# richardshuai/ExPecto

Measured on AMD Instinct MI355X. Metric: variants/sec (200 windows × 2002 feats) at 1/2/4/8 MI355X; HBM GB/s vs peak, higher is better.
Workload: dtype fp32 in/out (f16x3: power-of-2-scaled 2-way fp16 split = 22-bit operands, 3 MFMA products, fp32 accumulate; bf16x6 recompute on fp16 overflow)

## Files before the change

### expecto_amd/csrc/beluga.hip

```cpp
#include <hip/hip_runtime.h>

#include <algorithm>
#include <array>
#include <cstdint>
#include <cstdlib>
#include <cstring>
#include <map>
#include <memory>
#include <mutex>
#include <tuple>
#include <string>
#include <vector>

#include "beluga_knobs.h"
#include "common.h"
#include "event_pairs.h"
#include "gemm_kernel.h"
#include "seg_plan.h"

namespace expecto {

static_assert(kStrandFwd == EXPECTO_STRAND_FWD && kStrandRc == EXPECTO_STRAND_RC && kStrandBoth == EXPECTO_STRAND_BOTH &&
              EXPECTO_EINVAL == -1, "seg_plan.h restates the strand modes and the refusal code");
constexpr int kNFeat = 2002;
// ... 155 lines not shown
#pragma unroll
        for (int j = 0; j < 4; ++j) {
          const float v = fmaxf(fmaf(acc[rb][cb][j], sc[cb], bb[cb]), 0.f);
          vmax = fmaxf(vmax, v);
          _Float16 h, l;
          split_h2p(v, h, l);
          char* d = sw + (16 * rb + 4 * fq + j) * C1H_WROW + (cb >> 1) * 128 + ((cb & 1) * 16 + fr) * 2;
          *reinterpret_cast<_Float16*>(d) = h;
          *reinterpret_cast<_Float16*>(d + 64) = l;
        }
    asm volatile("s_waitcnt lgkmcnt(0)" ::: "memory");
#pragma unroll
    for (int i = 0; i < (C1H_STEP * 16) / 64; ++i) {
      const int k = i * 64 + lane, row = k >> 4, ch = k & 15;
      if (s + row < tend) {
        char* g = reinterpret_cast<char*>(out) + ((win * out_rows + t0 + s + row) * 10 + 2 * wave) * 128 + ch * 16;
        *reinterpret_cast<floatx4*>(g) = *reinterpret_cast<const floatx4*>(sw + row * C1H_WROW + ch * 16);
      }
    }
    asm volatile("s_waitcnt lgkmcnt(0)" ::: "memory");
  }
  if ((bad || !(vmax < 65504.f)) && ovf) *ovf = 1;
}

__global__ void fc1_reduce(const float* __restrict__ part, int splits, long long split_stride, long long count,
                           const float* __restrict__ bias, float* __restrict__ h1, int fmt,
                           const float* __restrict__ col_scale, float osc, int* __restrict__ ovf) {
  const long long i = (long long)blockIdx.x * blockDim.x + threadIdx.x;
  if (i >= count) return;
  const long long row = i / kHidLd;
  const int n = (int)(i - row * kHidLd);
  float s = 0.f;
  for (int k = 0; k < splits; ++k) s += part[k * split_stride + i];
  if (col_scale) s *= col_scale[n];
  const float v = n < kFc1Out ? fmaxf(s + bias[n], 0.f) : 0.f;
  store_act_rt(fmt, h1, row, kHidLd, n, v, osc, ovf);
}

typedef _Float16 halfx4 __attribute__((ext_vector_type(4)));
__global__ void fc1_reduce_h2(const float* __restrict__ part, int splits, long long split_stride, long long count4,
                              const float* __restrict__ bias, float* __restrict__ h1,
                              const float* __restrict__ col_scale, float osc, int* __restrict__ ovf) {
  const long long i4 = (long long)blockIdx.x * blockDim.x + threadIdx.x;
  if (i4 >= count4) return;
  const long long i = i4 * 4;
  const long long row = i / kHidLd;
  const int n = (int)(i - row * kHidLd);
  floatx4 s = {0.f, 0.f, 0.f, 0.f};
  for (int k = 0; k < splits; ++k) {
    const floatx4 v = *reinterpret_cast<const floatx4*>(part + k * split_stride + i);
#pragma unroll
    for (int e = 0; e < 4; ++e) s[e] += v[e];
  }
  halfx4 hv, lv;
  bool bad = false;
#pragma unroll
  for (int e = 0; e < 4; ++e) {
    float t = s[e];
    if (col_scale) t *= col_scale[n + e];
    const float v = n + e < kFc1Out ? fmaxf(t + bias[min(n + e, kFc1Out - 1)], 0.f) : 0.f;
    const float x = v * osc;
    bad |= !(fabsf(x) < 65504.f);
    _Float16 hh, ll;
    split_h2p(x, hh, ll);
    hv[e] = hh;
    lv[e] = ll;
  }
  if (bad && ovf) *ovf = 1;
  _Float16* d = reinterpret_cast<_Float16*>(h1) + act_index<2>(row, kHidLd, n);
  *reinterpret_cast<halfx4*>(d) = hv;
  *reinterpret_cast<halfx4*>(d + 32) = lv;
}

constexpr int kFc2Chunk = 8;
__device__ __forceinline__ float fc2_value(float s, const float* __restrict__ col_scale, const float* __restrict__ bias,
                                           int n) {
  if (col_scale) s *= col_scale[n];
  const float v = s + bias[n];
  return 1.0f / (1.0f + expf(-v));
}
__global__ __launch_bounds__(256) void fc2_reduce(const float* __restrict__ part, int splits, long long split_stride,
                                                  int M, const float* __restrict__ bias,
                                                  const float* __restrict__ col_scale,
                                                  const long long* __restrict__ c_rows, float* __restrict__ y) {
  static_assert(kNFeat % 2 == 0 && kHidLd % 2 == 0, "2 features per thread");
  const int n = 2 * (blockIdx.x * blockDim.x + threadIdx.x);
  if (n >= kNFeat) return;
  for (long long m = blockIdx.y; m < M; m += gridDim.y) {
    const float* src = part + m * kHidLd + n;
    float s0 = 0.f, s1 = 0.f;
    for (int k0 = 0; k0 < splits; k0 += kFc2Chunk) {
      float2 v[kFc2Chunk];
#pragma unroll
      for (int u = 0; u < kFc2Chunk; ++u)
        v[u] = *reinterpret_cast<const float2*>(src + (long long)min(k0 + u, splits - 1) * split_stride);
#pragma unroll
      for (int u = 0; u < kFc2Chunk; ++u)
        if (k0 + u < splits) {
          s0 += v[u].x;
          s1 += v[u].y;
        }
    }
    float2 o;
    o.x = fc2_value(s0, col_scale, bias, n);
    o.y = fc2_value(s1, col_scale, bias, n + 1);
    *reinterpret_cast<float2*>(y + (c_rows ? c_rows[m] : m) * kNFeat + n) = o;
  }
}
__global__ void fc2_reduce1(const float* __restrict__ part, int splits, long long split_stride, int M,
                            const float* __restrict__ bias, const float* __restrict__ col_scale,
                            const long long* __restrict__ c_rows, float* __restrict__ y) {
  const long long i = (long long)blockIdx.x * blockDim.x + threadIdx.x;
  if (i >= (long long)M * kNFeat) return;
  const int m = (int)(i / kNFeat), n = (int)(i - (long long)m * kNFeat);
  const long long src = (long long)m * kHidLd + n;
  float s = 0.f;
  for (int k = 0; k < splits; ++k) s += part[k * split_stride + src];
  y[(c_rows ? c_rows[m] : m) * kNFeat + n] = fc2_value(s, col_scale, bias, n);
}

__global__ void pool4_phases(const float* __restrict__ in, int n_seg, int s_in, int t_in, int C,
                             int n_ph, int4 ph, int s_out, float* __restrict__ out, int fmt) {
  const int c = threadIdx.x;
  const int g = blockIdx.x;
  const int i = blockIdx.y % n_ph;
  const long long seg = blockIdx.y / n_ph;
  const int p = i == 0 ? ph.x : i == 1 ? ph.y : i == 2 ? ph.z : ph.w;
  if (c >= C || g >= (t_in - p) / 4) return;
  const long long r0 = seg * s_in + p + 4LL * g, orow = (seg * n_ph + i) * s_out + g;
  float m = load_act_rt(fmt, in, r0, C, c);
#pragma unroll
  for (int j = 1; j < 4; ++j) m = fmaxf(m, load_act_rt(fmt, in, r0 + j, C, c));
  store_act_rt(fmt, out, orow, C, c, m);
}

typedef _Float16 halfx8 __attribute__((ext_vector_type(8)));
__global__ __launch_bounds__(256) void pool4_phases_h2(const float* __restrict__ in, int s_in, int t_in, int C,
                                                        int n_ph, int4 ph, int s_out, float* __restrict__ out) {
  const int c8 = threadIdx.x & 63;
  const int g = blockIdx.x * 4 + (threadIdx.x >> 6);
  const int i = blockIdx.y % n_ph;
  const long long seg = blockIdx.y / n_ph;
  const int p = i == 0 ? ph.x : i == 1 ? ph.y : i == 2 ? ph.z : ph.w;
  if (c8 >= C / 8 || g >= (t_in - p) / 4) return;
  const long long rb = (long long)C * 4;
  const int cofs = (c8 >> 2) * 128 + (c8 & 3) * 16;
  const char* src = reinterpret_cast<const char*>(in) + (seg * s_in + p + 4LL * g) * rb + cofs;
  halfx8 hi[4], lo[4];
#pragma unroll
  for (int j = 0; j < 4; ++j) {
    hi[j] = *reinterpret_cast<const halfx8*>(src + j * rb);
    lo[j] = *reinterpret_cast<const halfx8*>(src + j * rb + 64);
  }
  halfx8 oh, ol;
#pragma unroll
  for (int e = 0; e < 8; ++e) {
    float m = (float)hi[0][e] + (float)lo[0][e];
#pragma unroll
    for (int j = 1; j < 4; ++j) m = fmaxf(m, (float)hi[j][e] + (float)lo[j][e]);
    _Float16 h, l;
    split_h2(m, h, l);
    oh[e] = h;
    ol[e] = l;
  }
  char* dst = reinterpret_cast<char*>(out) + ((seg * n_ph + i) * s_out + g) * rb + cofs;
  *reinterpret_cast<halfx8*>(dst) = oh;
  *reinterpret_cast<halfx8*>(dst + 64) = ol;
}

__global__ __launch_bounds__(256) void pool4_phases_h2m(const float* __restrict__ in, int s_in, int t_in, int C,
                                                         int n_ph, int4 ph, int s_out, float* __restrict__ out) {
  const int c8 = threadIdx.x & 63;
  const int g = blockIdx.x * 4 + (threadIdx.x >> 6);
  const long long seg = blockIdx.y;
  const int pmin = ph.x;
  const int pmax = n_ph == 1 ? ph.x : n_ph == 2 ? ph.y : n_ph == 3 ? ph.z : ph.w;
  if (c8 >= C / 8 || g >= (t_in - pmin) / 4) return;
  const long long rb = (long long)C * 4;
  const int cofs = (c8 >> 2) * 128 + (c8 & 3) * 16;
  const char* src = reinterpret_cast<const char*>(in) + (seg * s_in + pmin + 4LL * g) * rb + cofs;
  const int nr = min(pmax - pmin + 4, t_in - pmin - 4 * g);
  halfx8 hi[7], lo[7];
#pragma unroll
  for (int j = 0; j < 7; ++j) {
    if (j < nr) {
      hi[j] = *reinterpret_cast<const halfx8*>(src + j * rb);
      lo[j] = *reinterpret_cast<const halfx8*>(src + j * rb + 64);
    }
  }
  float fv[7][8];
#pragma unroll
  for (int j = 0; j < 7; ++j)
#pragma unroll
    for (int e = 0; e < 8; ++e) fv[j][e] = j < nr ? (float)hi[j][e] + (float)lo[j][e] : 0.f;
#pragma unroll
  for (int i = 0; i < 4; ++i) {
    if (i >= n_ph) break;
    const int p = i == 0 ? ph.x : i == 1 ? ph.y : i == 2 ? ph.z : ph.w;
    if (g >= (t_in - p) / 4) continue;
    const int o = p - pmin;
    halfx8 oh, ol;
// ... 1557 lines not shown
      beluga_conv_h3p<4, EPI_POOL_PH02, 256, 4><<<dim3((unsigned)nblk), dim3(512), 0, st>>>(a);
    if ((rc = check_launch("beluga_conv_h3p pool2"))) return rc;
  }
  Timer lt(h, 3, st);
  if (a.m_tiles > 1)
    pool2_tile_seams<<<dim3((unsigned)(a.m_tiles - 1)), dim3(64), 0, st>>>(h->seam, a.M, s_in, t4, s5, dst);
  return check_launch("pool2_tile_seams");
}

float* h1_rows(expecto_beluga* h, long long rows) { return h->h1 + rows * kHidLd * act_bytes() / 4; }

bool fc_wide_tiles(const expecto_beluga* h) { return h->fc_wide && g_precision == EXPECTO_PRECISION_F16X3; }

bool fc1_narrow(const expecto_beluga* h, long long mtt);
bool fc_skinny(const expecto_beluga* h, long long rows);

int run_fc1(expecto_beluga* h, const float* act, const long long* a_rows, int nb, float* h1, hipStream_t st,
            const unsigned* ks_mask = nullptr, double slab_frac = 1.0, long long part_rows = 0) {
  if (part_rows <= 0) part_rows = nb;
  int rc;
  const long long m_tiles = (nb + gemm_bm() - 1) / gemm_bm();
  const bool wide = fc_wide_tiles(h);
  const int n_tiles1 = wide ? (kHidLd + FCW_BN - 1) / FCW_BN : npad_of(kFc1Out) / GBN;
  const int splits = h->fc_splits;
  {
    GemmArgs a{};
    a.A = act;
    a.a_rows = a_rows;
    a.lda = (long long)kFc1In;
    a.M = nb;
    a.B = h->fc1w;
    a.Bp = g_precision == EXPECTO_PRECISION_F16X3 ? h->wh[5] : h->fc1p;
    a.ldb = kFc1In;
    a.kper = kFc1In / splits;
    a.taps = 1;
    a.n_tiles = n_tiles1;
    a.m_tiles = m_tiles;
    a.m_fastest = (double)m_tiles * gemm_bm() * (kFc1In / splits) * 4.0 <= h->fc1_m_order_mb * (1 << 20) ? 1 : 0;
    a.linear_order = a.m_fastest;
    if (h->fc1_order == 2 && !a.m_fastest && m_tiles % 8 == 0 && planes_gemm() && g_precision == EXPECTO_PRECISION_F16X3)
      a.m_fastest = 2;
    if (h->fc1_order == 3 && g_precision == EXPECTO_PRECISION_F16X3) {
      a.m_fastest = 3;
      a.m_group = h->fc1_m_group;
      a.linear_order = 0;
    }
    if (wide) {
      a.m_fastest = 0;
      a.linear_order = 0;
      a.n_tile_cols = FCW_BN;
      if (!ks_mask && fc_skinny(h, nb)) {
        a.n_tile_cols = 16 * FCS_NB;
        a.n_tiles = kHidLd / a.n_tile_cols;
      } else if (!ks_mask && fc1_narrow(h, m_tiles * splits)) {
        a.n_tile_cols = 112;
        a.n_tiles = kHidLd / 112;
      }
    }
    a.C = h->part;
    a.ldc = kHidLd;
    a.n_store = kHidLd;
    a.split_stride = part_rows * kHidLd;
    a.ks_mask = ks_mask;
    EXPECTO_REQUIRE(!ks_mask || planes_gemm(), "slab mask needs the planes GEMM");
    Timer lt(h, 6, st);
    if (h->profiling) h->macs[h->timer_base + 6] += (double)nb * kFc1Out * kFc1In * slab_frac;
    if ((rc = launch_gemm<7, EPI_PARTIAL>(a, splits, st))) return rc;
  }
  {
    Timer lt(h, 7, st);
    const long long count = (long long)nb * kHidLd;
    const bool f16 = g_precision == EXPECTO_PRECISION_F16X3;
    if (act_fmt() == 2)
      fc1_reduce_h2<<<dim3((unsigned)((count / 4 + 255) / 256)), dim3(256), 0, st>>>(
          h->part, splits, part_rows * kHidLd, count / 4, h->fc1b, h1, h->cs[5], exp2i(h->sx[6]), h->ovf);
    else
      fc1_reduce<<<dim3((unsigned)((count + 255) / 256)), dim3(256), 0, st>>>(
          h->part, splits, part_rows * kHidLd, count, h->fc1b, h1, act_fmt(), f16 ? h->cs[5] : nullptr, exp2i(h->sx[6]), h->ovf);
    if ((rc = check_launch("fc1_reduce"))) return rc;
  }
  return EXPECTO_OK;
}

int run_fc2(expecto_beluga* h, const float* h1, int nb, float* y, hipStream_t st, const long long* c_rows) {
  int rc;
  const long long m_tiles = (nb + gemm_bm() - 1) / gemm_bm();
  {
    GemmArgs a{};
    a.A = h1;
    a.lda = kHidLd;
    a.M = nb;
    a.B = h->fc2w;
    a.Bp = g_precision == EXPECTO_PRECISION_F16X3 ? h->wh[6] : h->fc2p;
    a.col_scale = g_precision == EXPECTO_PRECISION_F16X3 ? h->cs[6] : nullptr;
    a.ldb = kHidLd;
    a.kper = kHidLd / h->fc2_splits;
    a.taps = 1;
    const bool wide = fc_wide_tiles(h) && h->fc2_splits > 1;
    a.n_tiles = wide ? (kNFeat + FCW_BN - 1) / FCW_BN : npad_of(kNFeat) / GBN;
    a.m_tiles = m_tiles;
    a.m_fastest = (double)m_tiles * gemm_bm() * (kHidLd / h->fc2_splits) * 4.0 <= h->fc1_m_order_mb * (1 << 20) ? 1 : 0;
    if (wide) {
      a.m_fastest = 0;
      a.n_tile_cols = FCW_BN;
      if (fc_skinny(h, nb)) {
        a.n_tile_cols = 16 * FCS_NB;
        a.n_tiles = (kNFeat + a.n_tile_cols - 1) / a.n_tile_cols;
      } else if (fc1_narrow(h, m_tiles * h->fc2_splits)) {
        a.n_tile_cols = 112;
        a.n_tiles = (kNFeat + 111) / 112;
      }
    }
    a.C = h->part2;
    a.ldc = kHidLd;
    a.n_store = kNFeat;
    a.split_stride = (long long)nb * kHidLd;
    Timer lt(h, 8, st);
    if (h->profiling) h->macs[h->timer_base + 8] += (double)nb * kNFeat * kFc1Out;
    if (h->fc2_splits == 1) {
      a.C = y;
      a.ldc = kNFeat;
      a.c_rows = c_rows;
      a.bias = h->fc2b;
      a.s_in = a.t_valid = a.s_out = 1;
      return launch_gemm<8, EPI_SIGMOID>(a, 1, st);
    }
    if ((rc = launch_gemm<8, EPI_PARTIAL>(a, h->fc2_splits, st))) return rc;
    if ((reinterpret_cast<uintptr_t>(y) & 7) == 0)
      fc2_reduce<<<dim3((unsigned)((kNFeat / 2 + 255) / 256), (unsigned)std::max<long long>(1, std::min<long long>(nb, 65535))), dim3(256), 0,
                   st>>>(h->part2, h->fc2_splits, (long long)nb * kHidLd, nb, h->fc2b, a.col_scale, c_rows, y);
    else
      fc2_reduce1<<<dim3((unsigned)(((long long)nb * kNFeat + 255) / 256)), dim3(256), 0, st>>>(
          h->part2, h->fc2_splits, (long long)nb * kHidLd, nb, h->fc2b, a.col_scale, c_rows, y);
    if ((rc = check_launch("fc2_reduce"))) return rc;
  }
  return EXPECTO_OK;
}

int run_fc(expecto_beluga* h, const float* act, const long long* a_rows, int nb, float* y, hipStream_t st,
           const long long* c_rows = nullptr, const unsigned* ks_mask = nullptr, double slab_frac = 1.0,
           long long part_rows = 0) {
  int rc;
  if ((rc = run_fc1(h, act, a_rows, nb, h->h1, st, ks_mask, slab_frac, part_rows))) return rc;
  return run_fc2(h, h->h1, nb, y, st, c_rows);
}

int count_desc_macs(expecto_beluga* h, const unsigned* mask, int tiles, double per_tile, hipStream_t st);

bool fk_use(const expecto_beluga* h) {
  return h->fk_on && h->fkw && g_precision == EXPECTO_PRECISION_F16X3 && h->fk_role < 4;
}
bool fk_use_seg(const expecto_beluga* h) { return h->fk_on && h->fkw && g_precision == EXPECTO_PRECISION_F16X3; }

int fk_cap(const expecto_beluga* h) {
  const long long dflt = std::min<long long>((long long)kFkSlicePerBatch * h->max_batch, 1LL << 30);
  return std::max(h->max_batch, h->fk_slice ? h->fk_slice : (int)dflt);
}
constexpr int kGresPerBatch = 3;

int fk_tables(expecto_beluga* h) {
  if (h->fk_grows) return EXPECTO_OK;
  const size_t mb = h->max_batch, tiles = (mb + 255) / 256, cap = fk_cap(h);
  float *a = nullptr, *b = nullptr, *c = nullptr, *d = nullptr;
  int rc;
  if ((rc = dalloc(h, &a, 2 * 9 * cap)) || (rc = dalloc(h, &b, 2 * mb)) || (rc = dalloc(h, &c, kFkParts * cap)) ||
      (rc = dalloc(h, &d, kFkParts * tiles)))
    return rc;
  h->fk_grows = reinterpret_cast<long long*>(a);
  h->fk_wrows = reinterpret_cast<long long*>(b);
  h->fk_prow = reinterpret_cast<int*>(c);
  h->fk_mask = reinterpret_cast<unsigned*>(d);
  return EXPECTO_OK;
}

int fk_seg_buffers(expecto_beluga* h) {
  if (h->fk_part) return EXPECTO_OK;
  const size_t cap = fk_cap(h);
  float *a = nullptr, *b = nullptr;
  int rc;
  if ((rc = dalloc(h, &h->fk_part, (size_t)kFkParts * cap * kHidLd)) || (rc = dalloc(h, &h->fk_h1, act_alloc(cap * kHidLd))) ||
      (rc = dalloc(h, &a, 2 * cap)) || (rc = dalloc(h, &b, 2 * cap)))
    return rc;
  h->fk_arows = reinterpret_cast<long long*>(a);
  h->fk_crows = reinterpret_cast<long long*>(b);
  float *c = nullptr, *d = nullptr, *e = nullptr, *f = nullptr, *q = nullptr, *m = nullptr;
  if ((rc = dalloc(h, &c, 9 * cap)) || (rc = dalloc(h, &d, 2 * cap)) || (rc = dalloc(h, &e, 2 * cap)) ||
      (rc = dalloc(h, &f, kFkParts * cap)) || (rc = dalloc(h, &q, cap)) || (rc = dalloc(h, &m, 19 * (cap / 256 + 1))))
    return rc;
  h->fk_rgrp = reinterpret_cast<int*>(c);
  h->fk_ginfo = reinterpret_cast<int*>(d);
  h->fk_winfo = reinterpret_cast<int*>(e);
  h->fk_aprow = reinterpret_cast<int*>(f);
  h->fk_aperm = reinterpret_cast<int*>(q);
  h->fk_smask = reinterpret_cast<unsigned*>(m);
  return EXPECTO_OK;
}

int fk_seq_alloc(expecto_beluga* h, long long rows, int set = 0) {
  int rc = EXPECTO_OK;
  for (DevBuf<float>& b : set ? h->fk_aseq : h->fk_seq)
    if ((rc = b.reserve(((size_t)rows + 16) * 640, h->bytes))) break;
  return rc;
}

int fk_sequences(expecto_beluga* h, const float* x, long long blocks, int T, int s, const int* tab, int n_ph,
                 hipStream_t st, const int* gres = nullptr, int set = 0) {
  int rc;
  if ((rc = fk_seq_alloc(h, blocks * s, set))) return rc;
  const DevBuf<float>* out = set ? h->fk_aseq : h->fk_seq;
  Timer lt(h, 7, st);
  const long long nblk = blocks * 7;
  EXPECTO_REQUIRE(nblk > 0 && nblk < (1LL << 31), "FC1 sequence grid");
  fk_seq_h2<<<dim3((unsigned)nblk), dim3(320), 0, st>>>(x, T, s, tab, n_ph, gres, out[0], out[1], out[2], h->ovf);
  return check_launch("fk_seq_h2");
}

// ... 266 lines not shown
  if ((rc = dalloc(h, &h->DA, act_alloc(da))) || (rc = dalloc(h, &h->D0, act_alloc(dd))) ||
      (rc = dalloc(h, &h->D1, act_alloc(dd))) || (rc = dalloc(h, &pc, (size_t)h->max_batch * kC1PatStride / 4)) ||
      (rc = dalloc(h, &tb, (size_t)h->max_batch * kSegTab)) ||
      (rc = dalloc(h, &h->slab_mask, (size_t)h->max_batch / 64 + 64)))
    return rc;
  h->delta_codes = reinterpret_cast<uint8_t*>(pc);
  h->seg_tab = reinterpret_cast<int*>(tb);
  if (h->overlap) {
    EXPECTO_HIP_CHECK(hipStreamCreateWithFlags(&h->st2, hipStreamNonBlocking));
    for (hipEvent_t& e : h->pev) EXPECTO_HIP_CHECK(hipEventCreateWithFlags(&e, hipEventDisableTiming));
  }
  return EXPECTO_OK;
}

struct SegPairs {
  const int* var_pos;
  const uint8_t* alt_code;
  float* y_alt;
  long long strand_stride;
};

struct SegCall {
  expecto_beluga* h;
  const SegPlan& pl;
  hipStream_t st, sa;
  const SegPairs* pr;
  SegDims gd;
  int4 ph4, phi;
  int eb;
  const uint8_t* codes;
  long long code_stride;
  int mode;
  float* y;
  const int* win_row_d;
};
struct SegChunk {
  size_t ci;
  int s0, ns, w0, nw;
  long long nb;
};
struct PQSwap {
  expecto_beluga* h;
  bool on;
  ~PQSwap() {
    if (on) std::swap(h->P, h->Q);
  }
};

int stream_order(hipStream_t from, hipStream_t to, hipEvent_t e) {
  if (from == to) return EXPECTO_OK;
  EXPECTO_HIP_CHECK(hipEventRecord(e, from));
  EXPECTO_HIP_CHECK(hipStreamWaitEvent(to, e, 0));
  return EXPECTO_OK;
}

int seg_alt_asm(const SegCall& c, const SegChunk& ck, int l, const float* ref, int ref_rows, const float* dprev,
                int wprev, int nbk, int ib, int mult, int irp, int arows, hipEvent_t ready, hipEvent_t done) {
  int rc;
  if ((rc = stream_order(c.st, c.sa, ready))) return rc;
  const int row16 = kConv[l].cin * c.eb / 16;
  seg_delta_assemble<<<dim3(ck.ns * nbk), dim3(256), 0, c.sa>>>(ref, ref_rows, dprev, wprev, c.h->seg_tab, nbk, ib,
                                                                 mult, irp, arows, row16, c.h->DA);
  rc = check_launch("seg_delta_assemble");
  if (!rc && c.sa != c.st) EXPECTO_HIP_CHECK(hipEventRecord(done, c.sa));
  return rc;
}
int seg_alt_gemm(const SegCall& c, const SegChunk& ck, int l, int nbk, int arows, int w, bool pool, float* dnext) {
  DeltaScope ds(c.h);
  return run_conv(c.h, l, c.h->DA, dnext, (long long)ck.ns * nbk, arows, w, w, pool, c.sa);
}
int seg_st_wait(const SegCall& c, hipEvent_t e) {
  if (c.sa != c.st) EXPECTO_HIP_CHECK(hipStreamWaitEvent(c.st, e, 0));
  return EXPECTO_OK;
}

int seg_rows(const SegCall& c, const SegChunk& ck, const int* widx, int w0, int n, long long* a_rows,
             long long* c_rows) {
  seg_a_rows<<<dim3((n + 255) / 256), dim3(256), 0, c.st>>>(c.h->win_seg_d, c.h->win_off_d, c.win_row_d, widx, w0, n,
                                                             ck.s0, c.pl.ss, c.pl.g.L, c.pl.n_ph, c.phi, c.pl.g.T6,
                                                             a_rows, c_rows);
  return check_launch("seg_a_rows");
}

int seg_fc2(const SegCall& c, const float* h1, int n, float* y, const long long* c_rows) {
  int rc;
  for (int r0 = 0; r0 < n; r0 += c.h->max_batch)
    if ((rc = run_fc2(c.h, h1 + (long long)r0 * kHidLd, std::min(c.h->max_batch, n - r0), y, c.st, c_rows + r0)))
      return rc;
  return EXPECTO_OK;
}

int seg_alt_conv6(const SegCall& c, const SegChunk& ck, bool on_sa = false) {
  int rc;
  const hipStream_t s = on_sa ? c.sa : c.st;
  if ((rc = s == c.st ? seg_st_wait(c, c.h->pev[13]) : stream_order(c.st, s, c.h->pev[14]))) return rc;
  seg_alt_blocks<<<dim3(kAltRows6, (unsigned)ck.nb), dim3(64), 0, s>>>(c.h->P, c.h->D0, c.pl.n_ph, c.pl.g.T6,
                                                                        c.h->seg_tab, 640 * c.eb / 16, c.h->Q);
  return check_launch("seg_alt_blocks");
}

int seg_copy_tail(const SegCall& c, const SegChunk& ck) {
  if (!c.pr) return EXPECTO_OK;
  const std::vector<int>& cw = c.pl.copy_w;
  const int ic0 = (int)(std::lower_bound(cw.begin(), cw.end(), ck.w0) - cw.begin());
  const int ic1 = (int)(std::lower_bound(cw.begin(), cw.end(), ck.w0 + ck.nw) - cw.begin());
  if (ic1 <= ic0) return EXPECTO_OK;
  copy_rows<<<dim3(ic1 - ic0), dim3(256), 0, c.st>>>(c.y, c.pr->y_alt, c.h->copy_w_d + ic0, c.win_row_d, c.pl.ss.n_win,
                                                      c.pl.ss.rc_rows);
  return check_launch("copy_rows");
}

int seg_trunk(const SegCall& c, const SegChunk& ck, PQSwap& pq) {
  expecto_beluga* h = c.h;
  const SegPairs* pr = c.pr;
  const SegGeo& g = c.pl.g;
  const hipStream_t st = c.st, sa = c.sa;
  const int s0 = ck.s0, ns = ck.ns, n_ph = c.pl.n_ph;
  const long long nb = ck.nb;
  int rc;
  if (pr && (rc = stream_order(st, sa, h->pev[0]))) return rc;
  const bool kmer = use_kmer(h, nullptr);
  const bool fuse = !kmer && fuse_conv1(h, nullptr);
  const C1Src f1{c.codes, c.code_stride, c.pl.ss.n_seg, c.mode, s0, g.L};
  if (!kmer && !fuse &&
      (rc = run_conv1(h, nullptr, c.codes, c.code_stride, c.pl.ss.n_seg, c.mode, s0, ns, g.L, g.S1, st)))
    return rc;
  if (pr) {
    seg_delta_table<<<dim3((ns + 255) / 256), dim3(256), 0, sa>>>(h->seg_var_d, s0, ns, c.pl.ss, c.gd, n_ph, c.ph4,
                                                                 h->seg_tab);
    if ((rc = check_launch("seg_delta_table"))) return rc;
    if (kmer || fuse) {
      seg_delta_codes2<<<dim3((ns + 4) / 5), dim3(5 * kC1PatStride), 0, sa>>>(
          c.codes, c.code_stride, pr->alt_code, s0, ns, c.pl.ss, g.L, h->seg_tab, h->delta_codes);
      if ((rc = check_launch("seg_delta_codes2"))) return rc;
      DeltaScope ds(h);
      if (fuse && (rc = run_conv1(h, nullptr, h->delta_codes, kC1PatStride, ns, EXPECTO_STRAND_FWD, 0, ns, kC1Pat,
                                  kDA[2], sa, h->DA)))
        return rc;
    } else {
      seg_delta_codes<<<dim3((ns + 15) / 16), dim3(256), 0, sa>>>(c.codes, c.code_stride, pr->alt_code, s0, ns,
                                                                 c.pl.ss, g.L, h->seg_tab, h->delta_codes);
      if ((rc = check_launch("seg_delta_codes"))) return rc;
      DeltaScope ds(h);
      if ((rc = run_conv1(h, nullptr, h->delta_codes, 16, ns, EXPECTO_STRAND_FWD, 0, ns, kDA[1], kDW[1], sa, h->D0)))
        return rc;
    }
  }
  if (pr && !kmer && !fuse &&
      (rc = seg_alt_asm(c, ck, 0, h->P, g.S1, h->D0, kDW[1], 1, 2, 4, 1, kDA[2], h->pev[1], h->pev[2])))
    return rc;
  if (kmer)
    rc = run_conv2_kmer(h, f1, ns, g.P1, g.P1, h->Q, st);
  else
    rc = run_conv(h, 0, h->P, h->Q, ns, g.S1, g.P1, g.P1, true, st, fuse ? &f1 : nullptr);
  if (rc) return rc;
  if (pr && kmer) {
    DeltaScope ds(h);
    const C1Src fa{h->delta_codes, kC1PatStride, ns, EXPECTO_STRAND_FWD, 0, kC1Pat};
    if ((rc = run_conv2_kmer(h, fa, ns, kDW[2], kDW[2], h->D1, sa))) return rc;
  } else if (pr && ((!fuse && (rc = seg_st_wait(c, h->pev[2]))) ||
                    (rc = seg_alt_gemm(c, ck, 0, 1, kDA[2], kDW[2], true, h->D1)))) {
    return rc;
  }
  if (pr && (rc = seg_alt_asm(c, ck, 1, h->Q, g.P1, h->D1, kDW[2], 1, 3, 1, 2, kDA[3], h->pev[3], h->pev[4])))
    return rc;
  const int T3p = (g.T3 + 3) & ~3;
  if ((rc = run_conv(h, 1, h->Q, h->P, ns, g.P1, g.T3, T3p, false, st))) return rc;
  if (pr && ((rc = seg_st_wait(c, h->pev[4])) || (rc = seg_alt_gemm(c, ck, 1, 1, kDA[3], kDW[3], false, h->D0))))
    return rc;
  if (pr && (rc = seg_alt_asm(c, ck, 2, h->P, T3p, h->D0, kDW[3], 1, 4, 1, 3, kA4u, h->pev[5], h->pev[6])))
    return rc;
// ... 123 lines not shown
  t.rows = row + (long long)ap.tail.size() - row0;
  const int fn = (int)(sl.i1 - sl.i0);
  for (int i = 0; i < fn; ++i) t.perm.push_back(ws[sl.i0 + i].w);
  auto pos_in = [](const std::vector<int>& l, int v) {
    const auto it = std::lower_bound(l.begin(), l.end(), v);
    return it != l.end() && *it == v ? (int)(it - l.begin()) : -1;
  };
  int k = -1;
  size_t next = 0;
  for (size_t i = 0; i < sl.nw_pre && next < ap.win.size(); ++i) {
    if (i == 0 || !fk_same_group(ws[sl.i0 + i], ws[sl.i0 + i - 1])) ++k;
    if ((int)i != ap.win[next]) continue;
    ++next;
    const FkWin& w = ws[sl.i0 + i];
    t.perm.push_back(w.w);
    const size_t p0 = prow.size();
    prow.resize(p0 + kFkParts);
    for (int j = 0; j < kFkParts; ++j) prow[p0 + j] = prow[i * kFkParts + j];
    for (int j = 0; j < 4; ++j) {
      const int g = kFkRole[fk_role_of(w.off6)][j];
      for (int sb = 0; sb < kFkSlabs; ++sb) {
        const int at = pos_in(ap.grp[g][sb], k);
        if (at >= 0) prow[p0 + kFkSlabs * j + sb] = (int)(base[g][sb] + at);
      }
    }
    const int at = pos_in(ap.tail, (int)i);
    if (at >= 0) prow[p0 + kFkParts - 1] = (int)(tail_base + at);
  }
  return t;
}

int seg_fc_karatsuba(const SegCall& c, const SegChunk& ck) {
  expecto_beluga* h = c.h;
  const SegPlan& pl = c.pl;
  const hipStream_t st = c.st;
  const int T6 = pl.g.T6, n_ph = pl.n_ph;
  const long long nb = ck.nb, cap = pl.fk_cap;
  const std::vector<FkWin>& ws = pl.fk_ref[ck.ci];
  const int* perm = h->fc_perm_d + ck.w0;
  int rc;
  const std::vector<int> gres = pl.fk_gres(ck.ci);
  EXPECTO_REQUIRE(nb <= kGresPerBatch * (long long)h->max_batch, "conv6 blocks of a chunk exceed fk_gres");
  if ((rc = stage_copies(h, {{h->fk_gres, gres.data(), gres.size() * sizeof(int)}}, st)) || (rc = fk_tables(h)) ||
      (rc = fk_seg_buffers(h)))
    return rc;
  bool alt_ready = false;
  const bool alt_early = c.pr && !h->fk_alt_inplace && !pl.fk_alt[ck.ci].empty();
  if (alt_early) {
    if ((rc = seg_alt_sequences(c, ck, true))) return rc;
    alt_ready = true;
  }
  if ((rc = fk_sequences(h, h->P, nb, T6, T6, nullptr, n_ph, st, h->fk_gres))) return rc;
  if (alt_early && (rc = seg_st_wait(c, h->pev[15]))) return rc;
  FkSlice sl{};
  for (size_t i0 = 0; i0 < ws.size(); i0 = sl.i1) {
    const char* refusal = pl.fk_slice(ck.ci, i0, sl);
    EXPECTO_REQUIRE(!refusal, refusal);
    const int fn = (int)(sl.i1 - i0);
    std::vector<long long> grows;
    std::vector<int> prow, rgrp, ginfo;
    FkProducts prd{h->fk_grows, {}, {}, {}};
    fk_slice_tables(ws, (int)i0, (int)sl.i1, T6, grows, prd, prow, &rgrp, &ginfo);
    if (sl.n_ag > 0 && !h->fk_alt_inplace) {
      const FkAltPlan ap = pl.fk_alt_plan(ck.ci, sl);
      const int na = (int)ap.win.size();
      long long ref_rows = fn, alt_lists = (long long)ap.tail.size();
      for (int g = 0; g < 9; ++g) {
        ref_rows += (long long)kFkSlabs * prd.cnt[g];
        for (int sb = 0; sb < kFkSlabs; ++sb) alt_lists += (long long)ap.grp[g][sb].size();
      }
      if (fn + na <= cap && ref_rows + alt_lists <= kFkParts * cap && (long long)grows.size() + alt_lists <= 9 * cap) {
        FkAltRowTables t = fk_alt_row_tables(ws, sl, ap, T6, ref_rows, grows, prow);
        t.ar.x = h->Q;
        t.ar.seq = h->fk_aseq;
        t.ar.g_rows = h->fk_grows;
        t.ar.w_rows = h->fk_grows + t.w_off;
        if ((rc = stage_copies(h, {{h->fk_grows, grows.data(), grows.size() * sizeof(long long)},
                                   {h->fk_prow, prow.data(), prow.size() * sizeof(int)},
                                   {h->fk_aperm, t.perm.data(), t.perm.size() * sizeof(int)}}, st)) ||
            (rc = seg_rows(c, ck, h->fk_aperm, 0, fn + na, h->fk_arows, h->fk_crows)) ||
            (rc = fk_fc1(h, h->P, h->fk_seq, prd, h->fk_arows, fn, nullptr, h->fk_h1, st, nullptr, 0, h->fk_part,
                         kFkParts * cap, &t.ar)) ||
            (rc = fk_reduce(h, h->fk_part, h->fk_prow, fn + na, h->fk_h1, st)) ||
            (rc = seg_fc2(c, h->fk_h1, fn, c.y, h->fk_crows)) ||
            (na > 0 && (rc = seg_fc2(c, h->fk_h1 + (long long)fn * kHidLd, na, c.pr->y_alt, h->fk_crows + fn))))
          return rc;
        continue;
      }
    }
    if ((rc = stage_copies(h, {{h->fk_grows, grows.data(), grows.size() * sizeof(long long)},
                               {h->fk_prow, prow.data(), prow.size() * sizeof(int)}}, st)) ||
        (rc = seg_rows(c, ck, perm + i0, 0, fn, h->fk_arows, h->fk_crows)) ||
        (rc = fk_fc1(h, h->P, h->fk_seq, prd, h->fk_arows, fn, h->fk_prow, h->fk_h1, st, nullptr, 0, h->fk_part,
                     kFkParts * cap)) ||
        (rc = seg_fc2(c, h->fk_h1, fn, c.y, h->fk_crows)))
      return rc;
    if (sl.n_ag == 0) continue;
    const FkAltTables t = fk_alt_tables(pl, ws, sl, prd, rgrp, prow);
    const int na = (int)t.aperm.size();
    const int tiles = (int)(cap / 256 + 1);
    if ((rc = stage_copies(h, {{h->fk_rgrp, rgrp.data(), rgrp.size() * sizeof(int)},
                               {h->fk_ginfo, ginfo.data(), ginfo.size() * sizeof(int)},
                               {h->fk_winfo, t.winfo.data(), t.winfo.size() * sizeof(int)},
                               {h->fk_aperm, t.aperm.data(), t.aperm.size() * sizeof(int)},
                               {h->fk_aprow, t.aprow.data(), t.aprow.size() * sizeof(int)}}, st)))
      return rc;
    if (!alt_ready) {
      if ((rc = seg_alt_sequences(c, ck, false))) return rc;
      alt_ready = true;
    }
    EXPECTO_HIP_CHECK(hipMemsetAsync(h->fk_smask, 0, (size_t)(t.md.n + 1) * tiles * sizeof(unsigned), st));
    int rows_max = t.md.nw;
    for (int i = 0; i < t.md.n; ++i) rows_max = std::max(rows_max, t.md.cnt[i]);
    if (rows_max > 0) {
      fk_seg_mask<<<dim3((rows_max + 255) / 256, t.md.n + 1), dim3(256), 0, st>>>(
          t.md, h->fk_rgrp, h->fk_ginfo, h->fk_winfo, h->seg_tab, n_ph, make_int4(0, 0, 0, 0), tiles, h->fk_smask);
      if ((rc = check_launch("fk_seg_mask"))) return rc;
    }
    DeltaScope ds(h);
    if ((rc = fk_fc1(h, h->Q, h->fk_aseq, t.pa, h->fk_arows, (int)sl.nw_pre, nullptr, h->fk_h1, st, h->fk_smask, tiles,
                     h->fk_part, kFkParts * cap)) ||
        (na > 0 && ((rc = fk_reduce(h, h->fk_part, h->fk_aprow, na, h->fk_h1, st)) ||
                    (rc = seg_rows(c, ck, h->fk_aperm, 0, na, h->fk_arows, h->fk_crows)) ||
                    (rc = seg_fc2(c, h->fk_h1, na, c.pr->y_alt, h->fk_crows)))))
      return rc;
  }
  return seg_copy_tail(c, ck);
}

int seg_fc_direct(const SegCall& c, const SegChunk& ck) {
  expecto_beluga* h = c.h;
  const SegPairs* pr = c.pr;
  const SegPlan& pl = c.pl;
  const hipStream_t st = c.st;
  const int w0 = ck.w0, nw = ck.nw;
  int rc;
  const int* widx = pr ? h->fc_perm_d + w0 : nullptr;
  const int n_alt = !pr ? 0 : (int)(std::lower_bound(pl.alt_w.begin(), pl.alt_w.end(), w0 + nw) -
                                    std::lower_bound(pl.alt_w.begin(), pl.alt_w.end(), w0));
  const bool gather2 = h->fc2_splits == 1;
  int pend = 0;
  auto flush2 = [&]() -> int {
    const int n2 = pend;
    pend = 0;
    return n2 ? run_fc2(h, h->h1, n2, c.y, st, h->c_rows) : EXPECTO_OK;
  };
  for (int f0 = 0; f0 < nw; f0 += h->max_batch) {
    const int fn = std::min(h->max_batch, nw - f0);
    if (gather2 && pend + fn > h->fc2_rows && (rc = flush2())) return rc;
    long long* crow = h->c_rows + (gather2 ? pend : 0);
    if ((rc = seg_rows(c, ck, widx ? widx + f0 : nullptr, w0 + f0, fn, h->a_rows, crow))) return rc;
    if (gather2) {
      if ((rc = run_fc1(h, h->P, h->a_rows, fn, h1_rows(h, pend), st))) return rc;
      pend += fn;
    } else if ((rc = run_fc(h, h->P, h->a_rows, fn, c.y, st, h->c_rows))) {
      return rc;
    }
    const int na = std::min(n_alt - f0, fn);
    if (na <= 0) continue;
    if (f0 == 0 && (rc = seg_alt_conv6(c, ck))) return rc;
    long long* acrow = gather2 ? h->c_rows + h->fc2_rows : h->c_rows;
    if ((rc = seg_rows(c, ck, widx + f0, 0, na, h->a_rows, acrow))) return rc;
    const unsigned* mask = nullptr;
    double frac = 1.0;
    if (planes_gemm()) {
      const int tiles = (int)((na + gemm_bm() - 1) / gemm_bm());
      unsigned* md = reinterpret_cast<unsigned*>(h->slab_mask);
      EXPECTO_HIP_CHECK(hipMemsetAsync(md, 0, tiles * sizeof(unsigned), st));
      fc1_slab_mask_seg<<<dim3((na + 255) / 256), dim3(256), 0, st>>>(
          widx + f0, na, h->win_seg_d, h->win_off_d, ck.s0, pl.ss, pl.g.L, c.phi, h->seg_tab, (int)gemm_bm(),
          kFc1In / h->fc_splits, md);
      if ((rc = check_launch("fc1_slab_mask_seg"))) return rc;
      mask = md;
      if (h->profiling) {
        if ((rc = count_slab_macs(h, md, tiles, na, st))) return rc;
        frac = 0.0;
      }
    }
    DeltaScope ds(h);
    if (gather2) {
      float* h1a = h1_rows(h, h->fc2_rows);
      if ((rc = run_fc1(h, h->Q, h->a_rows, na, h1a, st, mask, frac, fn)) ||
          (rc = run_fc2(h, h1a, na, pr->y_alt, st, acrow)))
        return rc;
    } else if ((rc = run_fc(h, h->Q, h->a_rows, na, pr->y_alt, st, h->c_rows, mask, frac, fn))) {
      return rc;
    }
  }
  if ((rc = flush2())) return rc;
  return seg_copy_tail(c, ck);
}

int forward_segments(expecto_beluga* h, const uint8_t* codes, int n_seg, int L, long long code_stride, int mode,
                     const int* win_seg, const int* win_off, const int* win_row, int n_win, float* y,
                     hipStream_t st, const SegPairs* pr = nullptr) {
  g_precision = h->precision;
  g_conv_ea = h->conv_ea;
  SegPlan pl;
  const char* refusal = nullptr;
  if (seg_plan({n_seg, L, mode, win_seg, win_off, win_row, n_win, pr ? pr->var_pos : nullptr,
                pr ? pr->strand_stride : n_win, h->max_batch, p_floats(h->max_batch) - 16 * 640,
                q_floats(h->max_batch) - 16 * 640, h->seg_merge_strands, h->seg_chunk_windows, fk_use_seg(h), fk_cap(h),
                h->fk_alt_inplace},
               pl, &refusal)) {
    set_error(refusal);
    return EXPECTO_EINVAL;
  }
// ... 702 lines not shown
```

### expecto_amd/csrc/beluga_knobs.h

```cpp
#pragma once

#include <algorithm>
#include <cstdlib>
#include <limits>

namespace expecto {

constexpr int kFc1KBlocks = 2120;
constexpr int kFc2KBlocks = 63;
constexpr int kFc2SplitsDefault = 7;
constexpr int kFcSplitsDefault = 8;

constexpr int kFkSlicePerBatch = 5;

struct BelugaKnobs {
  bool overlap = true;
  int fc_splits = kFcSplitsDefault;
  int fc2_splits = kFc2SplitsDefault;
  int fc2_rows_env = 0;
  double fc1_m_order_mb = 80.0;
  int fc1_order = 3;
  int fc1_m_group = 8;
  bool fc_wide = true;
  int conv_tile = 0;
  bool conv_ea = true;
  bool fc_skinny = true;
  int fc1_narrow = -1;
  int conv_narrow = -1;
  int seg_chunk_windows = 0;
  bool seg_merge_strands = true;
  bool pool_one_pass = true;
  bool pool_fused = true;
  bool fuse_conv1 = true;
  bool kmer_on = true;
  bool kmer_quad = true;
  double kmer_max_bytes = std::numeric_limits<double>::infinity();
  bool fk_on = true;
  int fk_role = 4;
  int fk_slice = 0;
  bool fk_alt_inplace = false;
  bool onehot_as_codes = true;
};

struct BelugaKnob {
  const char* name;
  bool BelugaKnobs::*b;
  int BelugaKnobs::*i;
  double BelugaKnobs::*d;
  int floor;
  bool (*ok)(int);
  const char* refusal;
};

namespace knob_detail {
using K = BelugaKnobs;
constexpr int kAny = std::numeric_limits<int>::min();
constexpr BelugaKnob flag(const char* n, bool K::*f) { return {n, f, nullptr, nullptr, kAny, nullptr, nullptr}; }
constexpr BelugaKnob num(const char* n, int K::*f, int floor = kAny, bool (*ok)(int) = nullptr, const char* why = nullptr) {
  return {n, nullptr, f, nullptr, floor, ok, why};
}
constexpr BelugaKnob real(const char* n, double K::*f) { return {n, nullptr, nullptr, f, kAny, nullptr, nullptr}; }
inline bool fc1_splits_ok(int v) { return v >= 1 && v <= 32 && kFc1KBlocks % v == 0; }
inline bool fc2_splits_ok(int v) { return v >= 1 && kFc2KBlocks % v == 0; }
inline bool role_ok(int v) { return v >= 0 && v <= 4; }
inline bool tri_ok(int v) { return v >= -1 && v <= 1; }
inline bool conv_tile_ok(int v) { return v == 0 || v == 256 || v == 384; }
}

inline constexpr BelugaKnob kBelugaKnobs[] = {
    knob_detail::num("EXPECTO_FC1_SPLITS", &BelugaKnobs::fc_splits, knob_detail::kAny, knob_detail::fc1_splits_ok,
                     "EXPECTO_FC1_SPLITS must divide 2120 and be <= 32"),
    knob_detail::num("EXPECTO_FC2_SPLITS", &BelugaKnobs::fc2_splits, knob_detail::kAny, knob_detail::fc2_splits_ok,
                     "EXPECTO_FC2_SPLITS must divide 63"),
    knob_detail::num("EXPECTO_FC2_ROWS", &BelugaKnobs::fc2_rows_env, 1),
    knob_detail::real("EXPECTO_FC1_M_ORDER_MB", &BelugaKnobs::fc1_m_order_mb),
    knob_detail::num("EXPECTO_FC1_ORDER", &BelugaKnobs::fc1_order),
    knob_detail::num("EXPECTO_FC1_M_GROUP", &BelugaKnobs::fc1_m_group, 1),
    knob_detail::flag("EXPECTO_FC_WIDE", &BelugaKnobs::fc_wide),
    knob_detail::flag("EXPECTO_OVERLAP", &BelugaKnobs::overlap),
    knob_detail::flag("EXPECTO_POOL_ONE_PASS", &BelugaKnobs::pool_one_pass),
    knob_detail::flag("EXPECTO_POOL_FUSED", &BelugaKnobs::pool_fused),
    knob_detail::flag("EXPECTO_FUSE_CONV1", &BelugaKnobs::fuse_conv1),
    knob_detail::flag("EXPECTO_CONV2_TABLE", &BelugaKnobs::kmer_on),
    knob_detail::flag("EXPECTO_KMER_QUAD", &BelugaKnobs::kmer_quad),
    knob_detail::real("EXPECTO_KMER_MAX_BYTES", &BelugaKnobs::kmer_max_bytes),
    knob_detail::flag("EXPECTO_ONEHOT_CODES", &BelugaKnobs::onehot_as_codes),
    knob_detail::flag("EXPECTO_FC1_KARATSUBA", &BelugaKnobs::fk_on),
    knob_detail::num("EXPECTO_FC1K_SLICE", &BelugaKnobs::fk_slice, 1),
    knob_detail::num("EXPECTO_FC1_ROLE", &BelugaKnobs::fk_role, knob_detail::kAny, knob_detail::role_ok,
                     "EXPECTO_FC1_ROLE must be 0..4"),
    knob_detail::num("EXPECTO_SEG_CHUNK_WINDOWS", &BelugaKnobs::seg_chunk_windows),
    knob_detail::flag("EXPECTO_SEG_MERGE_STRANDS", &BelugaKnobs::seg_merge_strands),
    knob_detail::num("EXPECTO_CONV_NARROW", &BelugaKnobs::conv_narrow, knob_detail::kAny, knob_detail::tri_ok,
                     "EXPECTO_CONV_NARROW must be -1 (auto), 0 or 1"),
    knob_detail::num("EXPECTO_FC1_NARROW", &BelugaKnobs::fc1_narrow, knob_detail::kAny, knob_detail::tri_ok,
                     "EXPECTO_FC1_NARROW must be -1 (auto), 0 or 1"),
    knob_detail::flag("EXPECTO_CONV_EA", &BelugaKnobs::conv_ea),
    knob_detail::flag("EXPECTO_FC_SKINNY", &BelugaKnobs::fc_skinny),
    knob_detail::num("EXPECTO_CONV_TILE", &BelugaKnobs::conv_tile, knob_detail::kAny, knob_detail::conv_tile_ok,
                     "EXPECTO_CONV_TILE must be 0 (auto), 256 or 384"),
};

inline constexpr BelugaKnob kBelugaSwitches[] = {
    knob_detail::flag("EXPECTO_FC1K_ALT_INPLACE", &BelugaKnobs::fk_alt_inplace),
};

template <class Getenv>
const char* beluga_knobs_parse(BelugaKnobs& k, Getenv&& get) {
  for (const BelugaKnob& s : kBelugaKnobs) {
    const char* e = get(s.name);
    if (!e) continue;
    if (s.b) {
      k.*s.b = atoi(e) != 0;
    } else if (s.d) {
      k.*s.d = atof(e);
    } else {
      const int v = std::max(s.floor, atoi(e));
      if (s.ok && !s.ok(v)) return s.refusal;
      k.*s.i = v;
    }
  }
  for (const BelugaKnob& s : kBelugaSwitches)
    if (const char* e = get(s.name)) k.*s.b = atoi(e) != 0;
  return nullptr;
}

}
```

### expecto_amd/csrc/seg_plan.h

```cpp
#pragma once

#include <algorithm>
#include <cstddef>
#include <map>
#include <tuple>
#include <utility>
#include <vector>

namespace expecto {

constexpr int kLen = 2000;
enum { kStrandFwd = 0, kStrandRc = 1, kStrandBoth = 2 };

struct SegStrands {
  int n_seg, rc_ent, n_win, rc_win;
  long long rc_rows;
};

struct SegGeo {
  int L, T1, S1, P1, T3, T4, S5, T5, T6;
  size_t p_rows_floats, q_rows_floats;
};

inline SegGeo seg_geo(int L, int n_ph) {
  SegGeo g{};
  g.L = L;
  g.T1 = L - 7;
  g.S1 = (g.T1 + 3) / 4 * 4;
  g.P1 = (g.T1 - 7) / 4;
  g.T3 = g.P1 - 7;
  g.T4 = g.T3 - 7;
  g.S5 = g.T4 / 4;
  g.T5 = g.S5 - 7;
  g.T6 = g.T5 - 7;
  const size_t p_conv1 = (size_t)g.S1 * 320, p_conv3 = (size_t)((g.T3 + 3) & ~3) * 480, p_pool2 = (size_t)n_ph * g.S5 * 480,
               p_conv6 = (size_t)n_ph * g.T6 * 640;
  const size_t q_pool1 = (size_t)g.P1 * 320, q_conv4 = (size_t)g.T4 * 480, q_conv5 = (size_t)n_ph * g.T5 * 640;
  g.p_rows_floats = std::max(std::max(p_conv1, p_conv3), std::max(p_pool2, p_conv6));
  g.q_rows_floats = std::max(q_pool1, std::max(q_conv4, q_conv5));
  return g;
}

struct FkWin {
  int w, blk, off6;
};
inline int fk_role_of(int off6) { return (off6 / 25) & 3; }
inline int fk_group_of(int off6) { return off6 - 25 * fk_role_of(off6); }
inline FkWin fk_win(int w, int seg, int off, bool rc, int L, int n_ph, const int* ph_idx) {
  const int o = rc ? L - kLen - off : off;
  const int q = o >> 2, p = q & 3;
  return {w, seg * n_ph + ph_idx[p], (q - p) >> 2};
}
inline bool fk_same_group(const FkWin& a, const FkWin& b) {
  return a.blk == b.blk && fk_group_of(a.off6) == fk_group_of(b.off6);
}

constexpr int kFkK = 16000;
constexpr int kFkSlabs = 2;
constexpr int kFkSeq[9] = {3, 2, 3, 1, 0, 1, 3, 2, 3};
constexpr int kFkBlk[9] = {0, 1, 1, 2, 3, 3, 2, 3, 3};
constexpr int kFkRole[4][4] = {{0, 1, 3, 4}, {1, 2, 4, 5}, {3, 4, 6, 7}, {4, 5, 7, 8}};

constexpr int kSegW[7] = {0, 8, 5, 12, 19, 6, 13};
constexpr int kSegW6 = 20;
inline int seg_floor4(int v) { return v >= 0 ? v >> 2 : -((3 - v) >> 2); }
inline int seg_clamp(int v, int lo, int hi) { return v < lo ? lo : (v > hi ? hi : v); }
inline int seg_r6(const SegGeo& g, int q, int p) {
  const int r1 = seg_clamp(q - 7, 0, g.T1 - kSegW[1]);
  const int r2 = seg_clamp(seg_floor4(r1 - 7), 0, g.P1 - kSegW[2]);
  const int r3 = seg_clamp(r2 - 7, 0, g.T3 - kSegW[3]);
  const int r4 = seg_clamp(r3 - 7, 0, g.T4 - kSegW[4]);
  const int r4p = seg_clamp(seg_floor4(r4 - p), 0, g.S5 - kSegW[5]);
  const int r5 = seg_clamp(r4p - 7, 0, g.T5 - kSegW[6]);
  return seg_clamp(r5 - 7, 0, g.T6 - kSegW6);
}

inline bool fk_reach(int G, int g, int s, int r6) {
  const int base = G + 25 * kFkBlk[g], per = kFkK / kFkSlabs;
  const int i0 = base + (s * per) / 640, i1 = base + ((s + 1) * per - 1) / 640;
  const int sq = kFkSeq[g], nl = sq == 0 ? 1 : sq == 3 ? 4 : 2, lag1 = sq == 2 ? 50 : 25;
  bool hit = false;
  for (int l = 0; l < nl; ++l) {
    const int lag = l == 0 ? 0 : (nl == 2 ? lag1 : 25 * l);
    hit |= i0 + lag < r6 + kSegW6 && i1 + lag >= r6;
  }
  return hit;
}
inline bool fk_reach_tail(int off6, int r6) { return off6 + 100 < r6 + kSegW6 && off6 + 105 >= r6; }

struct SegPlanIn {
  int n_seg, L, mode;
  const int *win_seg, *win_off, *win_row;
  int n_win;
  const int* var_pos;
  long long rc_rows;
  int max_batch;
  size_t p_cap, q_cap;
  bool merge_strands;
  int chunk_windows;
  bool fk;
  long long fk_cap;
  bool alt_inplace = false;
};

struct FkSlice {
  size_t i0, i1, nw_pre;
  int n_ag;
};

struct FkAltPlan {
  std::vector<int> grp[9][kFkSlabs];
  std::vector<int> win, tail;
};

struct SegPlan {
  int present[4], n_ph, ph[4], ph_idx[4];
  SegGeo g;
  int seg_cap;
  SegStrands ss;
  int n_ent, n_vw;
  int blk_per_seg;
  bool pairs;
  std::vector<int> first, vfirst;
  std::vector<char> is_alt;
  std::vector<int> alt_w, copy_w;
  std::vector<std::pair<int, int>> chunks;
  std::vector<int> fc_perm;
  bool fkm;
  std::vector<std::vector<FkWin>> fk_ref, fk_alt;
  long long fk_cap;
  bool alt_inplace;
  std::vector<int> r6;

  int vw_w(int v) const { return v >= ss.n_win ? v - ss.n_win : v; }
  bool v_is_alt(int v) const { return is_alt[vw_w(v)] != 0; }

  std::vector<int> fk_gres(size_t ci) const {
    std::vector<int> gres((size_t)(chunks[ci].second - chunks[ci].first) * n_ph, -2);
    for (const FkWin& w : fk_ref[ci]) {
      const int r = fk_group_of(w.off6) % 100;
      int& e = gres[(size_t)w.blk];
      e = e == -2 ? r : (e == r ? r : -1);
    }
    return gres;
  }

  const char* fk_slice(size_t ci, size_t i0, FkSlice& s) const {
    const std::vector<FkWin>& ws = fk_ref[ci];
    const bool twice = pairs && !alt_inplace && !fk_alt[ci].empty();
    size_t i1 = i0, rows = 0;
    while (i1 < ws.size()) {
      size_t j = i1, n = 0;
      do n += twice && v_is_alt(ws[j].w) ? 2 : 1;
      while (++j < ws.size() && fk_same_group(ws[j], ws[i1]));
      if (rows + n > (size_t)fk_cap && i1 > i0) break;
      rows += n;
      i1 = j;
    }
    if (i1 - i0 > (size_t)fk_cap) return "a Karatsuba FC1 window group exceeds the FC1 slice";
    s = {i0, i1, 0, 0};
    const bool has_alt = pairs && !fk_alt[ci].empty();
    for (size_t i = i0; has_alt && i < i1; ++i) {
      bool galt = false;
      size_t j = i;
      for (; j < i1 && fk_same_group(ws[j], ws[i]); ++j) galt |= v_is_alt(ws[j].w);
      if (!galt) break;
      ++s.n_ag;
      s.nw_pre = j - i0;
      i = j - 1;
    }
    return nullptr;
// ... 172 lines not shown
```

Measured before the change: 1547.

## Batch FC2 over ref and alt rows using the larger FC1 partial workspace

Runs FC2 for reference and alternate rows together, using the FC1-Karatsuba partial buffer as its split-K workspace instead of the smaller part2 buffer limited to max_batch. Rows are grouped into as few evenly sized passes as the workspace allows, and the reduce kernel routes each row to the primary or alternate output. The aim is fewer, larger GEMM and reduce launches with better tile occupancy. An env switch restores the old per-max_batch loop, and reusing fk_part assumes it is no longer needed once fk_reduce has run.

```diff
diff --git a/expecto_amd/csrc/beluga.hip b/expecto_amd/csrc/beluga.hip
--- a/expecto_amd/csrc/beluga.hip
+++ b/expecto_amd/csrc/beluga.hip
@@ -261,7 +261,8 @@
 __global__ __launch_bounds__(256) void fc2_reduce(const float* __restrict__ part, int splits, long long split_stride,
                                                   int M, const float* __restrict__ bias,
                                                   const float* __restrict__ col_scale,
-                                                  const long long* __restrict__ c_rows, float* __restrict__ y) {
+                                                  const long long* __restrict__ c_rows, float* __restrict__ y,
+                                                  int m_split, float* __restrict__ y2) {
   static_assert(kNFeat % 2 == 0 && kHidLd % 2 == 0, "2 features per thread");
   const int n = 2 * (blockIdx.x * blockDim.x + threadIdx.x);
   if (n >= kNFeat) return;
@@ -283,19 +284,20 @@
     float2 o;
     o.x = fc2_value(s0, col_scale, bias, n);
     o.y = fc2_value(s1, col_scale, bias, n + 1);
-    *reinterpret_cast<float2*>(y + (c_rows ? c_rows[m] : m) * kNFeat + n) = o;
+    *reinterpret_cast<float2*>((m < m_split ? y : y2) + (c_rows ? c_rows[m] : m) * kNFeat + n) = o;
   }
 }
 __global__ void fc2_reduce1(const float* __restrict__ part, int splits, long long split_stride, int M,
                             const float* __restrict__ bias, const float* __restrict__ col_scale,
-                            const long long* __restrict__ c_rows, float* __restrict__ y) {
+                            const long long* __restrict__ c_rows, float* __restrict__ y, int m_split,
+                            float* __restrict__ y2) {
   const long long i = (long long)blockIdx.x * blockDim.x + threadIdx.x;
   if (i >= (long long)M * kNFeat) return;
   const int m = (int)(i / kNFeat), n = (int)(i - (long long)m * kNFeat);
   const long long src = (long long)m * kHidLd + n;
   float s = 0.f;
   for (int k = 0; k < splits; ++k) s += part[k * split_stride + src];
-  y[(c_rows ? c_rows[m] : m) * kNFeat + n] = fc2_value(s, col_scale, bias, n);
+  (m < m_split ? y : y2)[(c_rows ? c_rows[m] : m) * kNFeat + n] = fc2_value(s, col_scale, bias, n);
 }
 
 __global__ void pool4_phases(const float* __restrict__ in, int n_seg, int s_in, int t_in, int C,
@@ -2019,8 +2021,13 @@
   return EXPECTO_OK;
 }
 
-int run_fc2(expecto_beluga* h, const float* h1, int nb, float* y, hipStream_t st, const long long* c_rows) {
+int run_fc2(expecto_beluga* h, const float* h1, int nb, float* y, hipStream_t st, const long long* c_rows,
+            float* ws = nullptr, int n_y = -1, float* y2 = nullptr) {
   int rc;
+  if (n_y < 0 || n_y > nb) n_y = nb;
+  EXPECTO_REQUIRE(ws || nb <= h->max_batch, "FC2 rows exceed its partial workspace");
+  EXPECTO_REQUIRE(n_y == nb || (y2 && h->fc2_splits != 1), "FC2 rows of a second output: split FC2 only");
+  if (!ws) ws = h->part2;
   const long long m_tiles = (nb + gemm_bm() - 1) / gemm_bm();
   {
     GemmArgs a{};
@@ -2048,7 +2055,7 @@
         a.n_tiles = (kNFeat + 111) / 112;
       }
     }
-    a.C = h->part2;
+    a.C = ws;
     a.ldc = kHidLd;
     a.n_store = kNFeat;
     a.split_stride = (long long)nb * kHidLd;
@@ -2063,12 +2070,12 @@
       return launch_gemm<8, EPI_SIGMOID>(a, 1, st);
     }
     if ((rc = launch_gemm<8, EPI_PARTIAL>(a, h->fc2_splits, st))) return rc;
-    if ((reinterpret_cast<uintptr_t>(y) & 7) == 0)
+    if (((reinterpret_cast<uintptr_t>(y) | reinterpret_cast<uintptr_t>(y2)) & 7) == 0)
       fc2_reduce<<<dim3((unsigned)((kNFeat / 2 + 255) / 256), (unsigned)std::max<long long>(1, std::min<long long>(nb, 65535))), dim3(256), 0,
-                   st>>>(h->part2, h->fc2_splits, (long long)nb * kHidLd, nb, h->fc2b, a.col_scale, c_rows, y);
+                   st>>>(ws, h->fc2_splits, (long long)nb * kHidLd, nb, h->fc2b, a.col_scale, c_rows, y, n_y, y2);
     else
       fc2_reduce1<<<dim3((unsigned)(((long long)nb * kNFeat + 255) / 256)), dim3(256), 0, st>>>(
-          h->part2, h->fc2_splits, (long long)nb * kHidLd, nb, h->fc2b, a.col_scale, c_rows, y);
+          ws, h->fc2_splits, (long long)nb * kHidLd, nb, h->fc2b, a.col_scale, c_rows, y, n_y, y2);
     if ((rc = check_launch("fc2_reduce"))) return rc;
   }
   return EXPECTO_OK;
@@ -2501,11 +2508,26 @@
   return check_launch("seg_a_rows");
 }
 
-int seg_fc2(const SegCall& c, const float* h1, int n, float* y, const long long* c_rows) {
+int seg_fc2(const SegCall& c, const float* h1, int n, float* y, int n_alt, float* y_alt, const long long* c_rows,
+            float* ws = nullptr, long long ws_rows = 0) {
+  expecto_beluga* h = c.h;
   int rc;
-  for (int r0 = 0; r0 < n; r0 += c.h->max_batch)
-    if ((rc = run_fc2(c.h, h1 + (long long)r0 * kHidLd, std::min(c.h->max_batch, n - r0), y, c.st, c_rows + r0)))
+  if (!ws || h->fc2_passes || h->fc2_splits == 1) {
+    for (int r0 = 0; r0 < n; r0 += h->max_batch)
+      if ((rc = run_fc2(h, h1 + (long long)r0 * kHidLd, std::min(h->max_batch, n - r0), y, c.st, c_rows + r0))) return rc;
+    for (int r0 = n; r0 < n + n_alt; r0 += h->max_batch)
+      if ((rc = run_fc2(h, h1 + (long long)r0 * kHidLd, std::min(h->max_batch, n + n_alt - r0), y_alt, c.st, c_rows + r0)))
+        return rc;
+    return EXPECTO_OK;
+  }
+  const Fc2Passes f = fc2_passes((long long)n + n_alt, ws_rows, h->fc2_splits);
+  EXPECTO_REQUIRE(f.passes > 0 || n + n_alt == 0, "FC2 workspace below one row per slab");
+  for (long long r0 = 0; r0 < n + n_alt; r0 += f.rows) {
+    const int nb = (int)std::min<long long>(f.rows, n + n_alt - r0);
+    const int n_y = (int)std::min<long long>(std::max<long long>(n - r0, 0), nb);
+    if ((rc = run_fc2(h, h1 + r0 * kHidLd, nb, n_y ? y : y_alt, c.st, c_rows + r0, ws, n_y ? n_y : nb, y_alt)))
       return rc;
+  }
   return EXPECTO_OK;
 }
 
@@ -2795,8 +2817,7 @@
             (rc = fk_fc1(h, h->P, h->fk_seq, prd, h->fk_arows, fn, nullptr, h->fk_h1, st, nullptr, 0, h->fk_part,
                          kFkParts * cap, &t.ar)) ||
             (rc = fk_reduce(h, h->fk_part, h->fk_prow, fn + na, h->fk_h1, st)) ||
-            (rc = seg_fc2(c, h->fk_h1, fn, c.y, h->fk_crows)) ||
-            (na > 0 && (rc = seg_fc2(c, h->fk_h1 + (long long)fn * kHidLd, na, c.pr->y_alt, h->fk_crows + fn))))
+            (rc = seg_fc2(c, h->fk_h1, fn, c.y, na, c.pr->y_alt, h->fk_crows, h->fk_part, kFkParts * cap)))
           return rc;
         continue;
       }
@@ -2806,7 +2827,7 @@
         (rc = seg_rows(c, ck, perm + i0, 0, fn, h->fk_arows, h->fk_crows)) ||
         (rc = fk_fc1(h, h->P, h->fk_seq, prd, h->fk_arows, fn, h->fk_prow, h->fk_h1, st, nullptr, 0, h->fk_part,
                      kFkParts * cap)) ||
-        (rc = seg_fc2(c, h->fk_h1, fn, c.y, h->fk_crows)))
+        (rc = seg_fc2(c, h->fk_h1, fn, c.y, 0, nullptr, h->fk_crows, sl.n_ag == 0 ? h->fk_part : nullptr, kFkParts * cap)))
       return rc;
     if (sl.n_ag == 0) continue;
     const FkAltTables t = fk_alt_tables(pl, ws, sl, prd, rgrp, prow);
@@ -2835,7 +2856,7 @@
                      h->fk_part, kFkParts * cap)) ||
         (na > 0 && ((rc = fk_reduce(h, h->fk_part, h->fk_aprow, na, h->fk_h1, st)) ||
                     (rc = seg_rows(c, ck, h->fk_aperm, 0, na, h->fk_arows, h->fk_crows)) ||
-                    (rc = seg_fc2(c, h->fk_h1, na, c.pr->y_alt, h->fk_crows)))))
+                    (rc = seg_fc2(c, h->fk_h1, 0, nullptr, na, c.pr->y_alt, h->fk_crows, h->fk_part, kFkParts * cap)))))
       return rc;
   }
   return seg_copy_tail(c, ck);
diff --git a/expecto_amd/csrc/beluga_knobs.h b/expecto_amd/csrc/beluga_knobs.h
--- a/expecto_amd/csrc/beluga_knobs.h
+++ b/expecto_amd/csrc/beluga_knobs.h
@@ -39,6 +39,7 @@
   int fk_role = 4;
   int fk_slice = 0;
   bool fk_alt_inplace = false;
+  bool fc2_passes = false;
   bool onehot_as_codes = true;
 };
 
@@ -103,6 +104,7 @@
 
 inline constexpr BelugaKnob kBelugaSwitches[] = {
     knob_detail::flag("EXPECTO_FC1K_ALT_INPLACE", &BelugaKnobs::fk_alt_inplace),
+    knob_detail::flag("EXPECTO_FC2_PASSES", &BelugaKnobs::fc2_passes),
 };
 
 template <class Getenv>
diff --git a/expecto_amd/csrc/seg_plan.h b/expecto_amd/csrc/seg_plan.h
--- a/expecto_amd/csrc/seg_plan.h
+++ b/expecto_amd/csrc/seg_plan.h
@@ -87,6 +87,19 @@
   return hit;
 }
 inline bool fk_reach_tail(int off6, int r6) { return off6 + 100 < r6 + kSegW6 && off6 + 105 >= r6; }
+
+struct Fc2Passes {
+  long long cap;
+  int passes;
+  long long rows;
+};
+inline Fc2Passes fc2_passes(long long n, long long ws_rows, int splits) {
+  Fc2Passes f{splits > 0 && ws_rows > 0 ? ws_rows / splits : 0, 0, 0};
+  if (n <= 0 || f.cap <= 0) return f;
+  f.passes = (int)((n + f.cap - 1) / f.cap);
+  f.rows = (n + f.passes - 1) / f.passes;
+  return f;
+}
 
 struct SegPlanIn {
   int n_seg, L, mode;
```

Result: no change. 1547 (-0.0%).
